# Desilo/liberate-fhe

Measured on AMD Instinct MI355X. Metric: NTTs/sec (forward negacyclic poly-NTT, logN=16, L=30 limbs, bit-exact vs reference semantics), higher is better.
Workload: dtype int64; 1 GPU; gold preset (logN=16), rows 9..38 of the prime chain (25 scale + base + 4 special primes = 30 limbs), 128 polynomials per GPU per step, forward NTT via lf_ntt_ws (C ABI: lf_ntt through a resident workspace of the operands' size); workspace_bytes=2013511680, batch_per_gpu=128, limbs=30, logN=16, parallelism=replicas x1 (independent polynomials)

## Files before the change

### include/ckks_hip.h

```cpp
#ifndef CKKS_HIP_H
#define CKKS_HIP_H

#include <stdint.h>

#ifdef __cplusplus
extern "C" {
#endif

#define LF_ERR_ARG 10001
#define LF_ERR_STATE 10002

#define LF_ABI_VERSION 15
int lf_abi_version(void);

#define LF_LIMIT_DIGIT_LIMBS 0
#define LF_LIMIT_SPECIAL_PRIMES 1
#define LF_LIMIT_ROWS 2
#define LF_LIMIT_BATCH 3
#define LF_LIMIT_LOGN 4
int lf_limits(int which);

#define LF_FP64_MAX_DIGITS 119

#define LF_BSGS_MAX_BABY_KEYS 63


#define LF_TUNE_KS_EXT_COLS_MAX 1
#define LF_TUNE_INTT_DIGITS 2
#define LF_TUNE_DIGIT_PLANES 3
#define LF_TUNE_WS_EXTRA_STAGE 4
#define LF_TUNE_MORE_PLANES 5
#define LF_TUNE_PC_MATMUL_TILE 6
int lf_tune(int which, int value);

int lf_clock_probe(uint64_t *out, int samples, uint64_t ticks, int device, void *stream);


int lf_mont_mult(const int64_t *a, const int64_t *b, int64_t *c, int rows, int64_t N,
                 const int64_t *ql, const int64_t *qh, const int64_t *kl, const int64_t *kh,
                 int device, void *stream);

int lf_mont_enter(int64_t *a, const int64_t *Rs, int rows, int64_t N,
                  const int64_t *ql, const int64_t *qh, const int64_t *kl, const int64_t *kh,
                  int device, void *stream);

int lf_mont_redc(int64_t *a, int rows, int64_t N,
                 const int64_t *ql, const int64_t *qh, const int64_t *kl, const int64_t *kh,
                 int device, void *stream);

int lf_reduce_2q(int64_t *a, int rows, int64_t N, const int64_t *_2q, int device, void *stream);
int lf_make_signed(int64_t *a, int rows, int64_t N, const int64_t *_2q, int device, void *stream);
int lf_make_unsigned(int64_t *a, int rows, int64_t N, const int64_t *_2q, int device, void *stream);
int lf_tile_unsigned(const int64_t *a, int64_t *dst, int rows, int64_t N, const int64_t *_2q,
                     int device, void *stream);
int lf_mont_add(const int64_t *a, const int64_t *b, int64_t *c, int rows, int64_t N, const int64_t *_2q,
// ... 347 lines not shown
```

### liberate_fhe_amd/csrc/ckks_common.h

```cpp
#pragma once
#include <hip/hip_runtime.h>
#include <stdint.h>

typedef long long i64;
typedef unsigned long long u64;
typedef unsigned __int128 u128;
typedef __int128 i128;

#define M62 ((1ull << 62) - 1ull)

#define KS_MAX_ALPHA 8
#define KS_MAX_K 8
#define MAX_LIST_ROWS 250
#define LF_BATCH_MAX 8
#define NTT_TILE_LOG_MAX 12
#define KS_LOGN_MAX (NTT_TILE_LOG_MAX + 5)


static __device__ __forceinline__ i64 mm62s(i64 a, i64 b, u64 q, u64 k) {
    const i128 x = (i128)a * (i128)b;
    const u64 lo = (u64)x;
    const i64 hi = (i64)(x >> 64);
    const u64 xl = lo & M62;
    const i64 xh = (i64)(((u64)hi << 2) | (lo >> 62));
// ... 80 lines not shown
#define DP_MAGIC 4503599627370496.0
static __device__ __forceinline__ double dp_from_word(i64 x) {
    return __longlong_as_double(x | 0x4330000000000000ll) - DP_MAGIC;
}
static __device__ __forceinline__ i64 dp_to_word(double d) {
    return __double_as_longlong(d + DP_MAGIC) & 0x000FFFFFFFFFFFFFll;
}

static __device__ __forceinline__ double dp_from_planes(unsigned lo, unsigned hi16) {
    return __longlong_as_double((i64)(((u64)(0x43300000u | hi16) << 32) | (u64)lo)) - DP_MAGIC;
}
typedef unsigned lf_u4_t __attribute__((ext_vector_type(4)));
typedef unsigned lf_u2_t __attribute__((ext_vector_type(2)));

static __device__ __forceinline__ double dp_from_signed(i64 x) {
    return __longlong_as_double(x + 0x4338000000000000ll) - 6755399441055744.0;
}


#define LF_FMT_RAW 0
#define LF_FMT_PLANES 1
#define LF_FMT_WS_SPLIT0 2
#define LF_FMT_WS_SPLIT1 3
void lf_fmt_note(const void *p, size_t bytes, int fmt);
void lf_fmt_epoch_bump(int fmt);
int lf_fmt_expect(const void *p, size_t bytes, int fmt);

static inline int lf_set_device(int device) {
    if (device >= 0) {
        hipError_t e = hipSetDevice(device);
        if (e != hipSuccess) return (int)e;
    }
    return 0;
}
```

### liberate_fhe_amd/csrc/ckks_hip.hip

```cpp
#include <mutex>
#include "../../include/ckks_hip.h"
#include "ckks_common.h"

namespace {


enum EwOp { EW_MULT, EW_ENTER, EW_REDC, EW_REDUCE, EW_SIGNED, EW_UNSIGNED, EW_TILE, EW_ADD, EW_SUB };

template <int OP>
__global__ void __launch_bounds__(256) ew_kernel(const i64 *a, const i64 *__restrict__ b, i64 *c,
                                                 i64 N, const i64 *__restrict__ v0, const i64 *__restrict__ ql,
                                                 const i64 *__restrict__ qh, const i64 *__restrict__ kl,
                                                 const i64 *__restrict__ kh) {
    const int row = blockIdx.y;
    const i64 j = ((i64)blockIdx.x * 256 + threadIdx.x) * 2;
    if (j >= N) return;
    const i64 off = (i64)row * N + j;
    u64 q = 0, k = 0;
    i64 q2 = 0, sc = 0;
    if (OP == EW_MULT || OP == EW_ENTER || OP == EW_REDC) {
        q = ((u64)qh[row] << 31) | (u64)ql[row];
        k = ((u64)kh[row] << 31) | (u64)kl[row];
    }
    if (OP == EW_ENTER) sc = v0[row];
// ... 79 lines not shown
        out[2 * i] = c1 - c0;
        out[2 * i + 1] = r1 - r0;
    }
}

}

namespace {
struct FmtRange {
    uintptr_t lo, hi;
    int fmt;
    unsigned long long age;
    unsigned epoch;
};
std::mutex g_fmt_mutex;
FmtRange g_fmt[256];
int g_fmt_n = 0;
unsigned long long g_fmt_clock = 0;
unsigned g_fmt_epoch[2] = {0, 0};
}

void lf_fmt_epoch_bump(int fmt) {
    std::lock_guard<std::mutex> lock(g_fmt_mutex);
    ++g_fmt_epoch[(fmt >> 1) & 1];
}

void lf_fmt_note(const void *p, size_t bytes, int fmt) {
    if (!p || !bytes) return;
    const uintptr_t lo = (uintptr_t)p, hi = lo + bytes;
    std::lock_guard<std::mutex> lock(g_fmt_mutex);
    int n = 0;
    for (int i = 0; i < g_fmt_n; ++i) {
        FmtRange r = g_fmt[i];
        if (r.hi <= lo || r.lo >= hi) {
            g_fmt[n++] = r;
            continue;
        }
        if (r.lo < lo) {
            r.hi = lo;
            g_fmt[n++] = r;
        } else if (r.hi > hi) {
            r.lo = hi;
            g_fmt[n++] = r;
        }
    }
    g_fmt_n = n;
    if (g_fmt_n == 256) {
        int o = 0;
        for (int i = 1; i < 256; ++i)
            if (g_fmt[i].age < g_fmt[o].age) o = i;
        g_fmt[o] = g_fmt[--g_fmt_n];
    }
    g_fmt[g_fmt_n++] = FmtRange{lo, hi, fmt, ++g_fmt_clock, g_fmt_epoch[(fmt >> 1) & 1]};
}

int lf_fmt_expect(const void *p, size_t bytes, int fmt) {
    if (!p || !bytes) return 0;
    const uintptr_t lo = (uintptr_t)p, hi = lo + bytes;
    std::lock_guard<std::mutex> lock(g_fmt_mutex);
    const int fam = (fmt >> 1) & 1;
    for (int i = 0; i < g_fmt_n; ++i)
        if (g_fmt[i].hi > lo && g_fmt[i].lo < hi && g_fmt[i].fmt != fmt && ((g_fmt[i].fmt >> 1) & 1) == fam &&
            g_fmt[i].epoch != g_fmt_epoch[fam])
            return LF_ERR_STATE;
    return 0;
}

extern "C" {

int lf_abi_version(void) { return LF_ABI_VERSION; }

int lf_clock_probe(uint64_t *out, int samples, uint64_t ticks, int device, void *stream) {
    if (!out || samples < 1 || samples > 4096 || ticks < 1 || ticks > 100000000ull || (uint64_t)samples * ticks > 1000000000ull)
        return LF_ERR_ARG;
    if (int e = lf_set_device(device)) return e;
    hipLaunchKernelGGL(clock_probe_kernel, dim3(1), dim3(64), 0, (hipStream_t)stream, (unsigned long long *)out, samples,
                       (unsigned long long)ticks);
    return (int)hipGetLastError();
}

int lf_limits(int which) {
    switch (which) {
        case LF_LIMIT_DIGIT_LIMBS: return KS_MAX_ALPHA;
        case LF_LIMIT_SPECIAL_PRIMES: return KS_MAX_K;
        case LF_LIMIT_ROWS: return MAX_LIST_ROWS;
// ... 91 lines not shown
```

### liberate_fhe_amd/csrc/ckks_ks.hip

```cpp
#include "../../include/ckks_hip.h"
#include "ckks_ntt_core.h"
#include "ckks_ntt_tile16.h"

#define KS_WORDS ((1 << NTT_TILE_LOG_MAX) / NTT_THREADS)

#define KS_ST(p, v)                                                  \
    do {                                                             \
        if (NT_KS_EXT) __builtin_nontemporal_store((i64)(v), p);     \
        else *(p) = (v);                                             \
    } while (0)

#define KS_ST_PL(rowb, N, idx, v)                                                                                \
    do {                                                                                                         \
        const i64 v_ = (i64)(v);                                                                                 \
        unsigned *lo_ = uniform_at(reinterpret_cast<unsigned *>(rowb) + (idx), lane);                            \
        unsigned short *hi_ = uniform_at(reinterpret_cast<unsigned short *>((rowb) + ((N) >> 1)) + (idx), lane); \
        if (NT_KS_EXT) {                                                                                         \
            __builtin_nontemporal_store((unsigned)v_, lo_);                                                      \
            __builtin_nontemporal_store((unsigned short)(v_ >> 32), hi_);                                        \
        } else {                                                                                                 \
            *lo_ = (unsigned)v_;                                                                                 \
            *hi_ = (unsigned short)(v_ >> 32);                                                                   \
        }                                                                                                        \
    } while (0)
// ... 3030 lines not shown
    }
    const dim3 grid((unsigned)((((i64)1 << logN) + 511) / 512), (unsigned)rows);
    const bool planes = key_format == LF_KEY_PLANES;
#define LF_BABYB_LAUNCH(NCT, PL, DPLB)                                                                                         \
    hipLaunchKernelGGL((ks_inner_babyb_kernel<NCT, PL, DPLB>), grid, dim3(256), 0, st, (const i64 *)ext, ba, (i64)part_stride, \
                       (i64)comp_stride, (i64)row_off, nparts, rows, logN, (const i64 *)ql, (const i64 *)qh, (const i64 *)kl,  \
                       (const i64 *)kh)
#define LF_BABYB_CASE(NCT)                                                                                                   \
    if (planes && dplanes) LF_BABYB_LAUNCH(NCT, true, true);                                                                 \
    else if (planes) LF_BABYB_LAUNCH(NCT, true, false);                                                                      \
    else if (dplanes) LF_BABYB_LAUNCH(NCT, false, true);                                                                     \
    else LF_BABYB_LAUNCH(NCT, false, false)
    if (nct == 2) {
        LF_BABYB_CASE(2);
    } else {
        LF_BABYB_CASE(4);
    }
#undef LF_BABYB_LAUNCH
#undef LF_BABYB_CASE
    return (int)hipGetLastError();
}

int lf_g_intt_digits = 1;
extern int lf_g_ws_extra_stage;

extern "C" {

int lf_tune(int which, int value) {
    int *knob = which == LF_TUNE_KS_EXT_COLS_MAX ? &g_ks_ext_cols_max : which == LF_TUNE_INTT_DIGITS ? &lf_g_intt_digits
                : which == LF_TUNE_DIGIT_PLANES ? &g_digit_planes : which == LF_TUNE_WS_EXTRA_STAGE ? &lf_g_ws_extra_stage
                : which == LF_TUNE_MORE_PLANES ? &g_more_planes : which == LF_TUNE_PC_MATMUL_TILE ? &g_pc_matmul_tile : nullptr;
    if (!knob) return -1;
    const int old = *knob;
    if (value < 0) return old;
    if (which == LF_TUNE_KS_EXT_COLS_MAX && value > 5) return old;
    if (which == LF_TUNE_MORE_PLANES && value > 3) return old;
    if (which == LF_TUNE_PC_MATMUL_TILE && value > 2) return old;
    if ((which == LF_TUNE_INTT_DIGITS || which == LF_TUNE_DIGIT_PLANES || which == LF_TUNE_WS_EXTRA_STAGE) && value > 1) return old;
    if (*knob != value && (which == LF_TUNE_DIGIT_PLANES || which == LF_TUNE_WS_EXTRA_STAGE || which == LF_TUNE_MORE_PLANES))
        lf_fmt_epoch_bump(which == LF_TUNE_WS_EXTRA_STAGE ? LF_FMT_WS_SPLIT0 : LF_FMT_RAW);
    *knob = value;
    return old;
}

int lf_key_planes(const int64_t *src_b, const int64_t *src_a, int64_t *dst_b, int64_t *dst_a, int rows, int64_t N,
                  const int64_t *ql, const int64_t *qh, int device, void *stream) {
    if (rows < 0 || rows > 65535 || N < 2 || (N & 1) || !src_b || !src_a || !dst_b || !dst_a || dst_b == dst_a || src_b == dst_b ||
        src_a == dst_a || src_a == dst_b || src_b == dst_a || !ql || !qh ||
        (((uintptr_t)src_b | (uintptr_t)src_a | (uintptr_t)dst_b | (uintptr_t)dst_a) & 15))
        return LF_ERR_ARG;
    if (rows == 0) return 0;
    if (int e = lf_set_device(device)) return e;
    hipLaunchKernelGGL(key_planes_kernel, dim3((unsigned)((N / 2 + 255) / 256), (unsigned)rows), dim3(256), 0, (hipStream_t)stream,
                       (const i64 *)src_b, (const i64 *)src_a, (i64 *)dst_b, (i64 *)dst_a, (i64)N, (const i64 *)ql, (const i64 *)qh);
    return (int)hipGetLastError();
}

int lf_ks_core_batch(const int64_t *state, int64_t state_stride, int nct, int nparts, int rows, int logN, const int64_t *desc,
                     const int64_t *E, const double *Ed, const int64_t *ksk, int64_t part_stride, int64_t comp_stride,
                     int64_t row_off, int key_format, int64_t *tmp, int64_t *s, const int64_t *psi_br, const double *psi_dp,
                     const int64_t *ipsi_br, const double *ipsi_dp, const int64_t *Ninv, const int64_t *q_host, const int64_t *ql, const int64_t *qh, const int64_t *kl, const int64_t *kh, int device,
                     void *stream) {
    if (nparts < 1 || rows < 1 || rows > MAX_LIST_ROWS || logN <= NTT_TILE_LOG_MAX || logN > KS_LOGN_MAX ||
// ... 98 lines not shown
```

### liberate_fhe_amd/csrc/ckks_ntt.hip

```cpp
#include <utility>
#include "../../include/ckks_hip.h"
#include "ckks_ntt_core.h"
#include "ckks_ntt_tile16.h"
#include <stdlib.h>

int lf_g_ws_extra_stage = 1;

namespace {

void classify(int rows, const int64_t *q_host, const void *dp_table, RowList &dp, RowList &in) {
    dp.n = in.n = 0;
    for (int r = 0; r < rows; ++r) {
        const bool small = q_host && dp_table && (uint64_t)q_host[r] < SMALL_PRIME_LIMIT;
        RowList &dst = small ? dp : in;
        dst.id[dst.n++] = (unsigned short)r;
    }
}

template <bool DP>
void launch_cols(int K, unsigned blocks, hipStream_t st, i64 *base, const PassGeom &g, const RowList &rl,
                 const int64_t *psi_br, const double *psi_dp, const i64 *rs, const int64_t *ql, const int64_t *qh,
                 const int64_t *kl, const int64_t *kh) {
#define LF_COLS_CASE(KK)                                                                                              \
    case KK:                                                                                                          \
        hipLaunchKernelGGL((ntt_fwd_cols<DP, KK>), dim3(blocks), dim3(NTT_COL_THREADS), 0, st, base, g, rl,           \
                           (const i64 *)psi_br, psi_dp, rs, (const i64 *)ql, (const i64 *)qh, (const i64 *)kl,        \
                           (const i64 *)kh);                                                                          \
        break;
    switch (K) {
// ... 254 lines not shown
    for (int pass = (S1 > 0 ? 0 : 1); pass < 2; ++pass) {
        if (only_pass && pass + 1 != only_pass) continue;
        PassGeom g = pass == 0 ? PassGeom{logN, tl, 1, S1, 0, tl - S1, rows, nb, relaxed, 0, plain}
                               : PassGeom{logN, tl, 0, tl, S1, 0, rows, nb, relaxed, 1, plain};
        const i64 *rs = (pass == 0 || S1 == 0) ? (const i64 *)Rs : nullptr;
        if (xpl) {
            const size_t bytes = ((size_t)nb * rows << logN) * 8;
            if (pass == 0) {
                g.pln = PLN_OUT;
                lf_fmt_note(base, bytes, LF_FMT_PLANES);
            } else if (int e = lf_fmt_expect(base, bytes, LF_FMT_PLANES)) {
                return e;
            }
        } else if (rsrc && relaxed && plain) {
            const size_t bytes = ((size_t)nb * rows << logN) * 8;
            if (pass == 0) lf_fmt_note(base, bytes, LF_FMT_RAW);
            else if (int e = lf_fmt_expect(base, bytes, LF_FMT_RAW)) return e;
        }
        if (through_ws) {
            const bool extra = lf_g_ws_extra_stage && S1 <= 4;
            const int Kc = S1 + (extra ? 1 : 0);
            {
                const size_t bytes = ((size_t)nb * rows << logN) * 8;
                const int fmt = extra ? LF_FMT_WS_SPLIT1 : LF_FMT_WS_SPLIT0;
                if (pass == 0) lf_fmt_note(ws, bytes, fmt);
                else if (int e = lf_fmt_expect(ws, bytes, fmt)) return e;
            }
            if (pass == 0) {
                const unsigned per_limb = (unsigned)nb * ((1u << (logN - Kc)) / NTT_COL_THREADS);
                const ClassLists cl = class_lists(in, dp, per_limb * (unsigned)in.n);
                const unsigned blocks = (unsigned)cl.in_blocks + per_limb * (unsigned)dp.n;
                switch (Kc) {
                    case 1: launch_cols_ws_k<1>(blocks, st, base, (i64 *)ws, wflags, g, cl, psi_br, psi_dp, rs, ql, qh, kl, kh); break;
                    case 2: launch_cols_ws_k<2>(blocks, st, base, (i64 *)ws, wflags, g, cl, psi_br, psi_dp, rs, ql, qh, kl, kh); break;
                    case 3: launch_cols_ws_k<3>(blocks, st, base, (i64 *)ws, wflags, g, cl, psi_br, psi_dp, rs, ql, qh, kl, kh); break;
                    case 4: launch_cols_ws_k<4>(blocks, st, base, (i64 *)ws, wflags, g, cl, psi_br, psi_dp, rs, ql, qh, kl, kh); break;
                    case 5: launch_cols_ws_k<5>(blocks, st, base, (i64 *)ws, wflags, g, cl, psi_br, psi_dp, rs, ql, qh, kl, kh); break;
                }
            } else {
                launch_pass16_ws(nb, st, (const i64 *)ws, wflags, base, g, in, dp, (const i64 *)psi_br, psi_dp, (const i64 *)ql,
                                 (const i64 *)qh, (const i64 *)kl, (const i64 *)kh, extra);
            }
            continue;
        }
        if (pass == 0 && (S1 <= 4 || (S1 == 5 && rsrc))) {
            const unsigned col_blocks = (unsigned)nb * ((1u << (logN - S1)) / NTT_COL_THREADS);
            if (rsrc) {
// ... 194 lines not shown
```

### liberate_fhe_amd/csrc/ckks_ntt_core.h

```cpp
#pragma once
#include "ckks_common.h"
#include <stdlib.h>

#define NTT_THREADS 512
#define NTT_PASS_WAVES 6
#define NTT_LDS_WORDS ((1 << NTT_TILE_LOG_MAX) + (1 << (NTT_TILE_LOG_MAX - 3)))
#define TAIL_NONE (-1)
#define SMALL_PRIME_LIMIT (1ull << 41)

#define PAD(L) ((L) + ((L) >> 3))
#define PAD_STRIDE(LOGDL) ((1 << (LOGDL)) + ((1 << (LOGDL)) >> 3))
#define NTT_FLAG_WORD NTT_LDS_WORDS

namespace {

__device__ __forceinline__ int lf_tid() {
    const int wave = __builtin_amdgcn_readfirstlane((int)threadIdx.x >> 6);
    int lane;
    asm volatile("v_mbcnt_lo_u32_b32 %0, -1, 0\n\tv_mbcnt_hi_u32_b32 %0, -1, %0" : "=v"(lane));
    return (wave << 6) | lane;
}

__device__ __forceinline__ void lds_barrier() {
    asm volatile("s_waitcnt lgkmcnt(0)" ::: "memory");
// ... 10 lines not shown
}

struct RowList {
    int n;
    unsigned short id[MAX_LIST_ROWS];
};

struct PassGeom {
    int logN;
    int tl;
    int strided;
    int S;
    int s0;
    int logC;
    int rows;
    int batch;
    int relaxed;
    int last;
    int plain;
    const unsigned char *skip_own;
    int skip_mod, skip_off;
    int pln;
    const i64 *pln_src;
};
#define PLN_IN 1
#define PLN_OUT 2

__device__ __forceinline__ int tile_gaddr(const PassGeom &g, int tile, int L) {
    if (!g.strided) return (tile << g.tl) + L;
    const int r = L >> g.logC, c = L & ((1 << g.logC) - 1);
    return (r << (g.logN - g.S)) + (tile << g.logC) + c;
}

__device__ __forceinline__ void block_coords(const PassGeom &g, const RowList &rl, int b, int &poly, int &limb, int &tile) {
    const int tiles = 1 << (g.logN - g.tl);
    const int pairs = rl.n * tiles;
    int pair;
    if ((pairs & 7) == 0) {
        const int x = b & 7, r = b >> 3;
        poly = r % g.batch;
        pair = (r / g.batch) * 8 + x;
    } else {
        pair = b / g.batch;
        poly = b % g.batch;
    }
    limb = rl.id[pair / tiles];
    tile = pair % tiles;
// ... 120 lines not shown
    const ShoupW *tw_sh;
    int relaxed;
    int inv_reduce;
};

template <bool DP>
__device__ __forceinline__ void set_aux(Ctx &c, const double *aux, int crow, int logN) {
    const double *row = aux ? aux + ((i64)crow << (logN + 1)) : nullptr;
    c.tw_dp = DP ? row : nullptr;
    c.tw_sh = DP ? nullptr : reinterpret_cast<const ShoupW *>(row);
}

template <bool SIGNED>
struct ArithInt {
    typedef i64 T;
    typedef i64 W;
    static __device__ __forceinline__ W tw(const Ctx &c, int idx) { return c.tw_mont[(unsigned)idx]; }
    template <int MAXC>
    static __device__ __forceinline__ void tw_group(const Ctx &c, int idx0, int cnt, W (&w)[MAXC]) { load_group<MAXC>(c.tw_mont, idx0, cnt, w); }
    static __device__ __forceinline__ T mul(const Ctx &c, W S, T O) {
        return SIGNED ? mm62s(S, O, c.m.q, c.m.k) : mm62u((u64)S, (u64)O, c.m.q, c.m.k);
    }
    static __device__ __forceinline__ void fwd(const Ctx &c, T &a, T &b, W S, int) {
        const T U = a, V = mul(c, S, b);
        if constexpr (SIGNED) {
            a = csub(U + V, c.m.q2);
            b = csub(U + c.m.q2 - V, c.m.q2);
        } else {
            a = (T)csub_u((u64)U + (u64)V, (u64)c.m.q2);
            b = (T)sub_lazy_u((u64)U, (u64)V, (u64)c.m.q2);
        }
    }
    static __device__ __forceinline__ void inv(const Ctx &c, T &a, T &b, W S, int) {
        const T U = a, V = b;
        if constexpr (SIGNED) {
            const T O = csub(U + c.m.q2 - V, c.m.q2);
            b = mul(c, S, O);
            a = csub(U + V, c.m.q2);
        } else {
            const T O = (T)sub_lazy_u((u64)U, (u64)V, (u64)c.m.q2);
            b = mul(c, S, O);
            a = (T)csub_u((u64)U + (u64)V, (u64)c.m.q2);
        }
    }
    template <int NN>
    static __device__ __forceinline__ void fwd_end(const Ctx &, T (&)[NN]) {}
    template <int NN>
// ... 918 lines not shown
                                                 unsigned char *__restrict__ wflags, const PassGeom &g, const RowList &rl,
                                                 const i64 *__restrict__ psi_br, const double *__restrict__ psi_dp,
                                                 const i64 *__restrict__ Rs, const i64 *__restrict__ ql,
                                                 const i64 *__restrict__ qh, const i64 *__restrict__ kl,
                                                 const i64 *__restrict__ kh) {
    constexpr int R = 1 << K;
    const int logC = g.logN - K;
    const int chunks = (1 << logC) / NTT_COL_THREADS;
    const int chunk = b % chunks, r = b / chunks;
    const int poly = __builtin_amdgcn_readfirstlane(r % g.batch), crow = __builtin_amdgcn_readfirstlane((int)rl.id[r / g.batch]);
    const bool enter = Rs != nullptr;
    Ctx c;
    c.m = load_mod(ql, qh, kl, kh, crow);
    c.tw_mont = psi_br + ((i64)crow << g.logN);
    set_aux<DP>(c, psi_dp, crow, g.logN);
    c.d = DP ? make_dp_tab(c.m, c.tw_dp) : make_dp(c.m);
    c.relaxed = 0;
    c.inv_reduce = 0;
    const i64 rs = enter ? Rs[crow] : 0;
    const i64 ri = (i64)(poly * g.rows + crow);
    const i64 col0 = (i64)chunk * NTT_COL_THREADS;
    const i64 *colu = a + (ri << g.logN) + col0;
    const unsigned lane = threadIdx.x;
    i64 w[R];
#pragma unroll
    for (int k = 0; k < R; ++k) w[k] = __builtin_nontemporal_load(uniform_at(colu + ((i64)k << logC), lane));
    int odd = 0;
#pragma unroll
    for (int k = 0; k < R; ++k) odd |= ((u64)w[k] >= (u64)c.m.q2);
    if (DP && !odd) {
        double x[R];
        const double r1 = enter ? (double)((1ull << 62) % c.m.q) : 0.0;
#pragma unroll
        for (int k = 0; k < R; ++k) {
            double v = dp_from_word(w[k]);
            if (enter) {
                v = dp_mulmod(v, r1, c.d);
                if (dp_below_fix_limit(v)) v = dp_lazy_fix(v, (u64)w[k], (u64)rs, c.d.q);
            }
            x[k] = v;
        }
        cols_fwd_stages<ArithDp, K>(x, c);
#pragma unroll
        for (int k = 0; k < R; ++k) w[k] = dp_to_word(dp_reduce(x[k], c.d.q2, c.d.q2inv));
    } else {
        if (enter) {
#pragma unroll
            for (int k = 0; k < R; ++k) {
                w[k] = mm62s(w[k], rs, c.m.q, c.m.k);
                odd |= ((u64)w[k] >= (u64)c.m.q2);
            }
        }
        if (odd || DP) cols_fwd_stages<ArithInt<true>, K>(w, c);
        else cols_fwd_stages<ArithInt<false>, K>(w, c);
    }
    i64 *orow = ws + (ri << g.logN);
    const bool wide = __builtin_amdgcn_ballot_w64(odd != 0) != 0;
    if ((lane & 63u) == 0) {
        const unsigned c0 = (unsigned)col0 + lane;
        wflags[(ri << 6) + (((c0 >> 6) & 3u) << 4) + (c0 >> 8)] = wide ? 1 : 0;
    }
    if constexpr (!DP) {
        const unsigned ls = lane_here(lane, orow);
#pragma unroll
        for (int k = 0; k < R; ++k) __builtin_nontemporal_store(w[k], uniform_at(orow + col0 + ((i64)k << logC), ls));
    } else {
        unsigned *lo = reinterpret_cast<unsigned *>(orow) + col0;
        unsigned short *mid = reinterpret_cast<unsigned short *>(orow + ((i64)1 << (g.logN - 1))) + col0;
#pragma unroll
        for (int k = 0; k < R; ++k) __builtin_nontemporal_store((unsigned)w[k], uniform_at(lo + ((i64)k << logC), lane));
#pragma unroll
        for (int k = 0; k < R; ++k)
            __builtin_nontemporal_store((unsigned short)((u64)w[k] >> 32), uniform_at(mid + ((i64)k << logC), lane));
        if (wide) {
            unsigned short *top = reinterpret_cast<unsigned short *>(orow + 3 * ((i64)1 << (g.logN - 2))) + col0;
#pragma unroll
            for (int k = 0; k < R; ++k) top[((i64)k << logC) + lane] = (unsigned short)((u64)w[k] >> 48);
// ... 480 lines not shown
```

### liberate_fhe_amd/csrc/ckks_ntt_tile16.h

```cpp
#pragma once
#include "ckks_ntt_core.h"

#define NTT16_THREADS 256
#define PAD16(L) ((L) + ((L) >> 4))
#define NTT16_LDS_WORDS (4096 + 256)
#define NTT16_FLAG NTT16_LDS_WORDS

namespace {

template <class A>
struct Tw16Early {
    typename A::W w1[1], w2[2], w4[4];
    __device__ __forceinline__ void load(const Ctx &c, int i) {
        A::tw_group(c, i, 1, w1);
        A::tw_group(c, i << 1, 2, w2);
        A::tw_group(c, i << 2, 4, w4);
    }
    __device__ __forceinline__ void get(int cnt, typename A::W (&wv)[8]) const {
#pragma unroll
        for (int j = 0; j < 4; ++j)
            if (j < cnt) wv[j] = cnt == 1 ? w1[0] : (cnt == 2 ? w2[j & 1] : w4[j]);
    }
};

template <class A>
struct Tw16Last {
    typename A::W w8[8];
    __device__ __forceinline__ void load(const Ctx &c, int i) { A::tw_group(c, i << 3, 8, w8); }
};

template <class A, int U0 = 0>
__device__ __forceinline__ void fwd_regs16(typename A::T (&x)[16], int i0, const Ctx &c, const Tw16Early<A> *early = nullptr,
                                           const Tw16Last<A> *last = nullptr) {
#pragma unroll
    for (int u = U0; u < 4; ++u) {
        const int du = 1 << (3 - u);
        typename A::W wv[8];
        if (early && u < 3) early->get(1 << u, wv);
        else if (last && u == 3) {
#pragma unroll
            for (int j = 0; j < 8; ++j) wv[j] = last->w8[j];
        } else A::tw_group(c, i0 << u, 1 << u, wv);
#pragma unroll
        for (int j = 0; j < (1 << u); ++j) {
            const int e0 = j << (4 - u);
#pragma unroll
            for (int t = 0; t < du; ++t) A::fwd(c, x[e0 + t], x[e0 + t + du], wv[j], (i0 << u) + j);
        }
    }
    A::fwd_end(c, x);
}

template <int U0 = 0>
__device__ __forceinline__ void fwd_regs16_exact(double (&x)[16], int i0, const Ctx &c, const Tw16Early<ArithDp> *early = nullptr,
                                                 const Tw16Last<ArithDp> *last = nullptr) {
#pragma unroll
    for (int u = U0; u < 4; ++u) {
        const int du = 1 << (3 - u);
        double wv[8];
        if (early && u < 3) early->get(1 << u, wv);
        else if (last && u == 3) {
#pragma unroll
            for (int j = 0; j < 8; ++j) wv[j] = last->w8[j];
        } else ArithDp::tw_group(c, i0 << u, 1 << u, wv);
        double V[8];
#pragma unroll
        for (int j = 0; j < (1 << u); ++j) {
            const int e0 = j << (4 - u);
#pragma unroll
            for (int t = 0; t < du; ++t) V[j * du + t] = dp_mulmod(x[e0 + t + du], wv[j], c.d);
        }
        int hmin = min(min(__double2hiint(V[0]), __double2hiint(V[1])), __double2hiint(V[2]));
        hmin = min(min(hmin, __double2hiint(V[3])), __double2hiint(V[4]));
        hmin = min(min(hmin, __double2hiint(V[5])), __double2hiint(V[6]));
        hmin = min(hmin, __double2hiint(V[7]));
        if (__builtin_expect(__builtin_amdgcn_ballot_w64(hmin < 0x41500000) != 0, 0)) {
#pragma unroll
            for (int j = 0; j < (1 << u); ++j) {
                const int e0 = j << (4 - u);
#pragma unroll
                for (int t = 0; t < du; ++t) {
// ... 63 lines not shown
                for (int t = 0; t < du; ++t) {
                    const int k = h * du + t;
                    if (dp_below_fix_limit(V[k]))
                        V[k] = dp_lazy_fix(V[k], (u64)c.tw_mont[(il << (3 - u)) + h], (u64)dp_reduce(O[k], c.d.q2, c.d.q2inv), c.d.q);
                }
            }
        }
#pragma unroll
        for (int h = 0; h < (1 << (3 - u)); ++h) {
            const int e0 = h << (u + 1);
#pragma unroll
            for (int t = 0; t < du; ++t) {
                const int k = h * du + t;
                x[e0 + t] = x[e0 + t] + x[e0 + t + du];
                x[e0 + t + du] = V[k];
            }
        }
    }
#pragma unroll
    for (int e = 0; e < 16; ++e) x[e] = dp_reduce(x[e], c.d.q2, c.d.q2inv);
}

__device__ __forceinline__ void tile16_slow_compute(i64 *sm, int base, int s0, int logN, bool inverse, const Ctx &c, int j0 = 0,
                                                    int j1 = 12) {
    for (int j = j0; j < j1; ++j) {
        const int st = s0 + j;
        const int logd = inverse ? j : 11 - j;
        for (int i = threadIdx.x; i < 2048; i += NTT16_THREADS) {
            const int pa = ((i >> logd) << (logd + 1)) | (i & ((1 << logd) - 1)), pb = pa + (1 << logd);
            i64 a = sm[PAD16(pa)], b = sm[PAD16(pb)];
            if (!inverse) {
                const int idx = (1 << st) + ((base + pa) >> (logN - st));
                ArithInt<true>::fwd(c, a, b, c.tw_mont[idx], idx);
            } else {
                const int idx = (1 << (logN - st - 1)) + ((base + pa) >> (st + 1));
                ArithInt<true>::inv(c, a, b, c.tw_mont[idx], idx);
            }
            sm[PAD16(pa)] = a;
            sm[PAD16(pb)] = b;
        }
        __syncthreads();
    }
}
__device__ __forceinline__ void tile16_slow_lds(i64 *sm, i64 *dst, int base, int s0, int logN, bool inverse, const Ctx &c, int j0 = 0,
                                                int j1 = 12) {
    tile16_slow_compute(sm, base, s0, logN, inverse, c, j0, j1);
    for (int L = threadIdx.x; L < 4096; L += NTT16_THREADS) dst[L] = sm[PAD16(L)];
}
__device__ __forceinline__ void tile16_slow(i64 *sm, const i64 *src, i64 *dst, int base, int s0, int logN, bool inverse, const Ctx &c) {
    for (int L = threadIdx.x; L < 4096; L += NTT16_THREADS) sm[PAD16(L)] = src[L];
    __syncthreads();
    tile16_slow_lds(sm, dst, base, s0, logN, inverse, c);
}

__device__ __forceinline__ void wave_flag_set16(i64 *sm, int pred, int w) {
    const bool any = __builtin_amdgcn_ballot_w64(pred != 0) != 0;
    if ((w & 63) == 0) reinterpret_cast<unsigned char *>(sm + NTT16_FLAG)[w >> 6] = any ? 1 : 0;
}
__device__ __forceinline__ bool tile_flagged16(const i64 *sm) { return reinterpret_cast<const unsigned *>(sm + NTT16_FLAG)[0] != 0; }

template <bool RLX> struct DpArith { typedef ArithDp type; };
template <> struct DpArith<true> { typedef ArithDpR type; };

template <class A, bool EXACT_DP, int U0 = 0>
__device__ __forceinline__ void fwd_step16(typename A::T (&x)[16], int i0, const Ctx &c, const Tw16Early<A> *early,
                                           const Tw16Last<A> *last = nullptr) {
    if constexpr (EXACT_DP) fwd_regs16_exact<U0>(x, i0, c, early, last);
    else fwd_regs16<A, U0>(x, i0, c, early, last);
}
template <class A, bool EXACT_DP>
__device__ __forceinline__ void inv_step16(typename A::T (&x)[16], int il, const Ctx &c, const Tw16Early<A> *early) {
    if constexpr (EXACT_DP) inv_regs16_exact(x, il, c, early);
    else inv_regs16<A>(x, il, c, early);
}

template <class A, bool DP, bool RLX, int U0 = 0>
__device__ __forceinline__ bool fwd_tile16_steps(typename A::T *smt, const i64 *sm, typename A::T (&x)[16], int w, int base,
                                                 int E, int s, const Ctx &c, bool check, const Tw16Last<A> *lastC = nullptr) {
    constexpr bool EX = DP && !RLX;
    const int iA = (1 << s) + (base >> (E - s));
    const int pB = ((w >> 4) << 8) | (w & 15);
    const int iB = (1 << (s + 4)) + ((base + pB) >> (E - s - 4));
    const int iC = (1 << (s + 8)) + ((base + 16 * w) >> (E - s - 8));
    Tw16Early<A> twB, twC;
    fwd_step16<A, EX, U0>(x, iA, c, nullptr);
    {
        typename A::T *sp = smt + PAD16(w);
#pragma unroll
        for (int e = 0; e < 16; ++e) sp[e * 272] = x[e];
    }
    twB.load(c, iB);
    lds_barrier();
    if (check && tile_flagged16(sm)) return false;
    {
        typename A::T *sp = smt + PAD16(pB);
#pragma unroll
        for (int e = 0; e < 16; ++e) x[e] = sp[e * 17];
        fwd_step16<A, EX>(x, iB, c, &twB);
#pragma unroll
        for (int e = 0; e < 16; ++e) sp[e * 17] = x[e];
    }
    twC.load(c, iC);
    lds_barrier();
    {
        const typename A::T *sp = smt + 17 * w;
#pragma unroll
        for (int e = 0; e < 16; ++e) x[e] = sp[e];
    }
// ... 127 lines not shown
            const unsigned l = __builtin_nontemporal_load(uniform_at(lo + (e << 8), (unsigned)w));
            const unsigned m = __builtin_nontemporal_load(uniform_at(mid + (e << 8), (unsigned)w));
            raw[e] = (i64)(((u64)m << 32) | (u64)l);
        }
        if ((fl | fh) != 0) {
            const unsigned short *top = reinterpret_cast<const unsigned short *>(srow + 3 * ((i64)1 << (E - 2))) + base;
#pragma unroll
            for (int e = 0; e < 16; ++e)
                if ((((e < 8 ? fl : fh) >> (8 * (e & 7))) & 0xffull) != 0) raw[e] |= (i64)((u64)top[(e << 8) + w] << 48);
        }
    } else {
#pragma unroll
        for (int e = 0; e < 16; ++e) raw[e] = __builtin_nontemporal_load(uniform_at(srow + base + (e << 8), (unsigned)w));
    }
    return (fl | fh) != 0;
}

template <bool DP, bool SKIP0>
__device__ __forceinline__ void fwd_tile16_ws(i64 *sm, const i64 *__restrict__ srow, const unsigned char *__restrict__ wf,
                                              i64 *__restrict__ row, int tile, const PassGeom &g, const Ctx &c,
                                              const Tw16Last<typename FwdArith<DP, false>::type> *lastC = nullptr) {
    const int w = lf_tid();
    const int base = tile << 12, E = g.logN, s = g.s0;
    i64 raw[16];
    const bool flagged = ws_load_tile<DP, SKIP0>(srow, wf, base, E, w, raw);
    {
        int odd = 0;
        if (flagged) {
#pragma unroll
            for (int e = 0; e < 16; ++e) odd |= ((u64)raw[e] >= (u64)c.m.q2);
        }
        wave_flag_set16(sm, odd, w);
    }
    i64 o[16];
    bool ok;
    if constexpr (DP) {
        double x[16];
#pragma unroll
        for (int e = 0; e < 16; ++e) x[e] = dp_from_word(raw[e]);
        ok = fwd_tile16_steps<ArithDp, true, false, SKIP0 ? 1 : 0>(reinterpret_cast<double *>(sm), sm, x, w, base, E, s, c, true, lastC);
#pragma unroll
        for (int e = 0; e < 16; ++e) o[e] = dp_to_word(dp_reduce(x[e], c.d.q2, c.d.q2inv));
    } else {
        ok = fwd_tile16_steps<ArithInt<false>, false, false, SKIP0 ? 1 : 0>(sm, sm, raw, w, base, E, s, c, true, lastC);
#pragma unroll
        for (int e = 0; e < 16; ++e) o[e] = raw[e];
    }
    if (!ok) {
        __syncthreads();
        ws_load_tile<DP, SKIP0>(srow, wf, base, E, w, raw);
#pragma unroll
        for (int e = 0; e < 16; ++e) sm[PAD16(w + (e << 8))] = raw[e];
        __syncthreads();
        tile16_slow_lds(sm, row + base, base, s, E, false, c, SKIP0 ? 1 : 0);
        return;
    }
    {
        i64 *sp = sm + 17 * w;
#pragma unroll
        for (int e = 0; e < 16; ++e) sp[e] = o[e];
    }
    wave_lds_sync();
    const int L0 = ((w >> 6) << 10) + ((w & 63) << 1);
    const i64 *so = sm + PAD16(L0);
#pragma unroll
    for (int i = 0; i < 8; ++i) {
        longlong2 v;
        v.x = so[i * 136];
        v.y = so[i * 136 + 1];
        if constexpr (NT_EXACT) nt_store2(row + base + L0 + (i << 7), v);
        else *reinterpret_cast<longlong2 *>(row + base + L0 + (i << 7)) = v;
    }
}

template <class A, bool DP, bool RLX>
__device__ __forceinline__ bool inv_tile16_steps(typename A::T *smt, const i64 *sm, typename A::T (&x)[16], int w, int base,
                                                 int logN, int s, const Ctx &c, bool check) {
// ... 448 lines not shown
    const u64 fl = fp[0], fh = SKIP0 ? fp[0] : fp[1];
    if constexpr (DP) {
        const unsigned *lo = reinterpret_cast<const unsigned *>(srow) + base;
        const unsigned short *mid = reinterpret_cast<const unsigned short *>(srow + ((i64)1 << (E - 1))) + base;
#pragma unroll
        for (int e = 0; e < 16; ++e) {
            pf.lo[e] = __builtin_nontemporal_load(uniform_at(lo + (e << 8), (unsigned)w));
            pf.mid[e] = __builtin_nontemporal_load(uniform_at(mid + (e << 8), (unsigned)w));
        }
    } else {
#pragma unroll
        for (int e = 0; e < 16; ++e) pf.raw[e] = __builtin_nontemporal_load(uniform_at(srow + base + (e << 8), (unsigned)w));
    }
    return (fl | fh) != 0;
}

template <bool DP, bool SKIP0>
__device__ __forceinline__ void fwd_tile16_ws_pf(i64 *sm, TilePf<DP> &pf, bool &pf_flagged, const i64 *__restrict__ srow,
                                                  const unsigned char *__restrict__ wf, i64 *__restrict__ row, int tile,
                                                  const PassGeom &g, const Ctx &c, const Tw16Last<typename FwdArith<DP, false>::type> *lastC,
                                                  const i64 *__restrict__ nsrow, const unsigned char *__restrict__ nwf, int ntile) {
    const int w = lf_tid();
    const int base = tile << 12, E = g.logN, s = g.s0;
    i64 raw[16];
    const bool flagged = pf_flagged;
    if (flagged) {
        ws_load_tile<DP, SKIP0>(srow, wf, base, E, w, raw);
    } else if constexpr (DP) {
#pragma unroll
        for (int e = 0; e < 16; ++e) raw[e] = (i64)(((u64)pf.mid[e] << 32) | (u64)pf.lo[e]);
    } else {
#pragma unroll
        for (int e = 0; e < 16; ++e) raw[e] = pf.raw[e];
    }
    {
        int odd = 0;
        if (flagged) {
#pragma unroll
            for (int e = 0; e < 16; ++e) odd |= ((u64)raw[e] >= (u64)c.m.q2);
        }
        wave_flag_set16(sm, odd, w);
    }
    i64 o[16];
    bool ok;
    if constexpr (DP) {
        double x[16];
#pragma unroll
        for (int e = 0; e < 16; ++e) x[e] = dp_from_word(raw[e]);
        ok = fwd_tile16_steps<ArithDp, true, false, SKIP0 ? 1 : 0>(reinterpret_cast<double *>(sm), sm, x, w, base, E, s, c, true, lastC);
#pragma unroll
        for (int e = 0; e < 16; ++e) o[e] = dp_to_word(dp_reduce(x[e], c.d.q2, c.d.q2inv));
    } else {
        ok = fwd_tile16_steps<ArithInt<false>, false, false, SKIP0 ? 1 : 0>(sm, sm, raw, w, base, E, s, c, true, lastC);
#pragma unroll
        for (int e = 0; e < 16; ++e) o[e] = raw[e];
    }
    if (!ok) {
        __syncthreads();
        ws_load_tile<DP, SKIP0>(srow, wf, base, E, w, raw);
#pragma unroll
        for (int e = 0; e < 16; ++e) sm[PAD16(w + (e << 8))] = raw[e];
        __syncthreads();
        tile16_slow_lds(sm, row + base, base, s, E, false, c, SKIP0 ? 1 : 0);
        if (ntile >= 0) pf_flagged = ws_prefetch_tile<DP, SKIP0>(nsrow, nwf, ntile << 12, E, w, pf);
        else pf = TilePf<DP>{};
        return;
    }

    {
        i64 *sp = sm + 17 * w;
#pragma unroll
        for (int e = 0; e < 16; ++e) sp[e] = o[e];
    }
    __builtin_amdgcn_sched_barrier(0);
    if (ntile >= 0) pf_flagged = ws_prefetch_tile<DP, SKIP0>(nsrow, nwf, ntile << 12, E, w, pf);
    else pf = TilePf<DP>{};
    __builtin_amdgcn_sched_barrier(0);
    wave_lds_sync();
    const int L0 = ((w >> 6) << 10) + ((w & 63) << 1);
    const i64 *so = sm + PAD16(L0);
#pragma unroll
    for (int i = 0; i < 8; ++i) {
        longlong2 v;
        v.x = so[i * 136];
        v.y = so[i * 136 + 1];
        if constexpr (NT_EXACT) nt_store2(row + base + L0 + (i << 7), v);
// ... 219 lines not shown
```

Before: 82460 poly-NTT/s.

## Premultiply extra-stage twiddles in column pass to skip tile's first twiddle multiply

When the workspace split includes an extra stage, the column pass now multiplies its outputs by the next stage's twiddle factors (both the DP and integer paths), so the tile16 pass can run its first butterfly stage as plain add/sub without a modular multiply. A new tune knob selects this per arithmetic path, and the workspace format tag encodes the premultiplied variant so stale workspaces are rejected. This moves the twiddle multiply from the register-heavy tile kernel into the column kernel, which adds twiddle loads and a fix-up path there.

Result: no change. 83180 poly-NTT/s (median of 3 runs) (+0.9%).

```diff
diff --git a/include/ckks_hip.h b/include/ckks_hip.h
--- a/include/ckks_hip.h
+++ b/include/ckks_hip.h
@@ -31,6 +31,7 @@
 #define LF_TUNE_WS_EXTRA_STAGE 4
 #define LF_TUNE_MORE_PLANES 5
 #define LF_TUNE_PC_MATMUL_TILE 6
+#define LF_TUNE_WS_PREMUL 7
 int lf_tune(int which, int value);
 
 int lf_clock_probe(uint64_t *out, int samples, uint64_t ticks, int device, void *stream);
diff --git a/liberate_fhe_amd/csrc/ckks_common.h b/liberate_fhe_amd/csrc/ckks_common.h
--- a/liberate_fhe_amd/csrc/ckks_common.h
+++ b/liberate_fhe_amd/csrc/ckks_common.h
@@ -126,6 +126,7 @@
 #define LF_FMT_PLANES 1
 #define LF_FMT_WS_SPLIT0 2
 #define LF_FMT_WS_SPLIT1 3
+#define LF_FMT_FAMILY(fmt) ((fmt) >= LF_FMT_WS_SPLIT0 ? 1 : 0)
 void lf_fmt_note(const void *p, size_t bytes, int fmt);
 void lf_fmt_epoch_bump(int fmt);
 int lf_fmt_expect(const void *p, size_t bytes, int fmt);
diff --git a/liberate_fhe_amd/csrc/ckks_hip.hip b/liberate_fhe_amd/csrc/ckks_hip.hip
--- a/liberate_fhe_amd/csrc/ckks_hip.hip
+++ b/liberate_fhe_amd/csrc/ckks_hip.hip
@@ -125,7 +125,7 @@
 
 void lf_fmt_epoch_bump(int fmt) {
     std::lock_guard<std::mutex> lock(g_fmt_mutex);
-    ++g_fmt_epoch[(fmt >> 1) & 1];
+    ++g_fmt_epoch[LF_FMT_FAMILY(fmt)];
 }
 
 void lf_fmt_note(const void *p, size_t bytes, int fmt) {
@@ -154,16 +154,16 @@
             if (g_fmt[i].age < g_fmt[o].age) o = i;
         g_fmt[o] = g_fmt[--g_fmt_n];
     }
-    g_fmt[g_fmt_n++] = FmtRange{lo, hi, fmt, ++g_fmt_clock, g_fmt_epoch[(fmt >> 1) & 1]};
+    g_fmt[g_fmt_n++] = FmtRange{lo, hi, fmt, ++g_fmt_clock, g_fmt_epoch[LF_FMT_FAMILY(fmt)]};
 }
 
 int lf_fmt_expect(const void *p, size_t bytes, int fmt) {
     if (!p || !bytes) return 0;
     const uintptr_t lo = (uintptr_t)p, hi = lo + bytes;
     std::lock_guard<std::mutex> lock(g_fmt_mutex);
-    const int fam = (fmt >> 1) & 1;
+    const int fam = LF_FMT_FAMILY(fmt);
     for (int i = 0; i < g_fmt_n; ++i)
-        if (g_fmt[i].hi > lo && g_fmt[i].lo < hi && g_fmt[i].fmt != fmt && ((g_fmt[i].fmt >> 1) & 1) == fam &&
+        if (g_fmt[i].hi > lo && g_fmt[i].lo < hi && g_fmt[i].fmt != fmt && LF_FMT_FAMILY(g_fmt[i].fmt) == fam &&
             g_fmt[i].epoch != g_fmt_epoch[fam])
             return LF_ERR_STATE;
     return 0;
diff --git a/liberate_fhe_amd/csrc/ckks_ks.hip b/liberate_fhe_amd/csrc/ckks_ks.hip
--- a/liberate_fhe_amd/csrc/ckks_ks.hip
+++ b/liberate_fhe_amd/csrc/ckks_ks.hip
@@ -3076,23 +3076,25 @@
 }
 
 int lf_g_intt_digits = 1;
-extern int lf_g_ws_extra_stage;
+extern int lf_g_ws_extra_stage, lf_g_ws_premul;
 
 extern "C" {
 
 int lf_tune(int which, int value) {
     int *knob = which == LF_TUNE_KS_EXT_COLS_MAX ? &g_ks_ext_cols_max : which == LF_TUNE_INTT_DIGITS ? &lf_g_intt_digits
                 : which == LF_TUNE_DIGIT_PLANES ? &g_digit_planes : which == LF_TUNE_WS_EXTRA_STAGE ? &lf_g_ws_extra_stage
-                : which == LF_TUNE_MORE_PLANES ? &g_more_planes : which == LF_TUNE_PC_MATMUL_TILE ? &g_pc_matmul_tile : nullptr;
+                : which == LF_TUNE_MORE_PLANES ? &g_more_planes : which == LF_TUNE_PC_MATMUL_TILE ? &g_pc_matmul_tile
+                : which == LF_TUNE_WS_PREMUL ? &lf_g_ws_premul : nullptr;
     if (!knob) return -1;
     const int old = *knob;
     if (value < 0) return old;
     if (which == LF_TUNE_KS_EXT_COLS_MAX && value > 5) return old;
-    if (which == LF_TUNE_MORE_PLANES && value > 3) return old;
+    if ((which == LF_TUNE_MORE_PLANES || which == LF_TUNE_WS_PREMUL) && value > 3) return old;
     if (which == LF_TUNE_PC_MATMUL_TILE && value > 2) return old;
     if ((which == LF_TUNE_INTT_DIGITS || which == LF_TUNE_DIGIT_PLANES || which == LF_TUNE_WS_EXTRA_STAGE) && value > 1) return old;
-    if (*knob != value && (which == LF_TUNE_DIGIT_PLANES || which == LF_TUNE_WS_EXTRA_STAGE || which == LF_TUNE_MORE_PLANES))
-        lf_fmt_epoch_bump(which == LF_TUNE_WS_EXTRA_STAGE ? LF_FMT_WS_SPLIT0 : LF_FMT_RAW);
+    const bool ws_knob = which == LF_TUNE_WS_EXTRA_STAGE || which == LF_TUNE_WS_PREMUL;
+    if (*knob != value && (which == LF_TUNE_DIGIT_PLANES || ws_knob || which == LF_TUNE_MORE_PLANES))
+        lf_fmt_epoch_bump(ws_knob ? LF_FMT_WS_SPLIT0 : LF_FMT_RAW);
     *knob = value;
     return old;
 }
diff --git a/liberate_fhe_amd/csrc/ckks_ntt.hip b/liberate_fhe_amd/csrc/ckks_ntt.hip
--- a/liberate_fhe_amd/csrc/ckks_ntt.hip
+++ b/liberate_fhe_amd/csrc/ckks_ntt.hip
@@ -5,6 +5,7 @@
 #include <stdlib.h>
 
 int lf_g_ws_extra_stage = 1;
+int lf_g_ws_premul = 1;
 
 namespace {
 
@@ -305,7 +306,8 @@
             const int Kc = S1 + (extra ? 1 : 0);
             {
                 const size_t bytes = ((size_t)nb * rows << logN) * 8;
-                const int fmt = extra ? LF_FMT_WS_SPLIT1 : LF_FMT_WS_SPLIT0;
+                g.ws_premul = extra ? (lf_g_ws_premul & 3) : 0;
+                const int fmt = extra ? LF_FMT_WS_SPLIT1 + g.ws_premul : LF_FMT_WS_SPLIT0;
                 if (pass == 0) lf_fmt_note(ws, bytes, fmt);
                 else if (int e = lf_fmt_expect(ws, bytes, fmt)) return e;
             }
diff --git a/liberate_fhe_amd/csrc/ckks_ntt_core.h b/liberate_fhe_amd/csrc/ckks_ntt_core.h
--- a/liberate_fhe_amd/csrc/ckks_ntt_core.h
+++ b/liberate_fhe_amd/csrc/ckks_ntt_core.h
@@ -56,7 +56,9 @@
     int skip_mod, skip_off;
     int pln;
     const i64 *pln_src;
+    int ws_premul;
 };
+__device__ __forceinline__ bool ws_premul_on(const PassGeom &g, bool dp) { return ((g.ws_premul >> (dp ? 0 : 1)) & 1) != 0; }
 #define PLN_IN 1
 #define PLN_OUT 2
 
@@ -223,7 +225,11 @@
         return SIGNED ? mm62s(S, O, c.m.q, c.m.k) : mm62u((u64)S, (u64)O, c.m.q, c.m.k);
     }
     static __device__ __forceinline__ void fwd(const Ctx &c, T &a, T &b, W S, int) {
-        const T U = a, V = mul(c, S, b);
+        b = mul(c, S, b);
+        fwd_sums(c, a, b);
+    }
+    static __device__ __forceinline__ void fwd_sums(const Ctx &c, T &a, T &b) {
+        const T U = a, V = b;
         if constexpr (SIGNED) {
             a = csub(U + V, c.m.q2);
             b = csub(U + c.m.q2 - V, c.m.q2);
@@ -1188,6 +1194,7 @@
     const i64 col0 = (i64)chunk * NTT_COL_THREADS;
     const i64 *colu = a + (ri << g.logN) + col0;
     const unsigned lane = threadIdx.x;
+    const bool premul = ws_premul_on(g, DP) && (((unsigned)col0 >> (logC - 1)) & 1u) != 0;
     i64 w[R];
 #pragma unroll
     for (int k = 0; k < R; ++k) w[k] = __builtin_nontemporal_load(uniform_at(colu + ((i64)k << logC), lane));
@@ -1207,8 +1214,38 @@
             x[k] = v;
         }
         cols_fwd_stages<ArithDp, K>(x, c);
-#pragma unroll
-        for (int k = 0; k < R; ++k) w[k] = dp_to_word(dp_reduce(x[k], c.d.q2, c.d.q2inv));
+        if (premul) {
+            constexpr int G = R < 8 ? R : 8;
+            double tw[G];
+            load_group<G>(c.tw_dp, R, G, tw);
+#pragma unroll
+            for (int k0 = 0; k0 < R; k0 += G) {
+                double tn[G], V[G];
+                if (k0 + G < R) load_group<G>(c.tw_dp, R + k0 + G, G, tn);
+                int hmin = 0x7fffffff;
+#pragma unroll
+                for (int j = 0; j < G; ++j) {
+                    V[j] = dp_mulmod(x[k0 + j], tw[j], c.d);
+                    hmin = min(hmin, __double2hiint(V[j]));
+                }
+                if (__builtin_expect(__builtin_amdgcn_ballot_w64(hmin < 0x41500000) != 0, 0)) {
+#pragma unroll
+                    for (int j = 0; j < G; ++j)
+                        if (dp_below_fix_limit(V[j]))
+                            V[j] = dp_lazy_fix(V[j], (u64)c.tw_mont[R + k0 + j], (u64)dp_reduce(x[k0 + j], c.d.q2, c.d.q2inv), c.d.q);
+                }
+#pragma unroll
+                for (int j = 0; j < G; ++j) {
+                    x[k0 + j] = V[j];
+                    if (k0 + G < R) tw[j] = tn[j];
+                }
+            }
+        } else {
+#pragma unroll
+            for (int k = 0; k < R; ++k) x[k] = dp_reduce(x[k], c.d.q2, c.d.q2inv);
+        }
+#pragma unroll
+        for (int k = 0; k < R; ++k) w[k] = dp_to_word(x[k]);
     } else {
         if (enter) {
 #pragma unroll
@@ -1217,8 +1254,19 @@
                 odd |= ((u64)w[k] >= (u64)c.m.q2);
             }
         }
-        if (odd || DP) cols_fwd_stages<ArithInt<true>, K>(w, c);
-        else cols_fwd_stages<ArithInt<false>, K>(w, c);
+        if (odd || DP) {
+            cols_fwd_stages<ArithInt<true>, K>(w, c);
+            if (premul) {
+#pragma unroll
+                for (int k = 0; k < R; ++k) w[k] = ArithInt<true>::mul(c, c.tw_mont[R + k], w[k]);
+            }
+        } else {
+            cols_fwd_stages<ArithInt<false>, K>(w, c);
+            if (premul) {
+#pragma unroll
+                for (int k = 0; k < R; ++k) w[k] = ArithInt<false>::mul(c, c.tw_mont[R + k], w[k]);
+            }
+        }
     }
     i64 *orow = ws + (ri << g.logN);
     const bool wide = __builtin_amdgcn_ballot_w64(odd != 0) != 0;
diff --git a/liberate_fhe_amd/csrc/ckks_ntt_tile16.h b/liberate_fhe_amd/csrc/ckks_ntt_tile16.h
--- a/liberate_fhe_amd/csrc/ckks_ntt_tile16.h
+++ b/liberate_fhe_amd/csrc/ckks_ntt_tile16.h
@@ -29,12 +29,22 @@
     __device__ __forceinline__ void load(const Ctx &c, int i) { A::tw_group(c, i << 3, 8, w8); }
 };
 
-template <class A, int U0 = 0>
+template <class A, int U0 = 0, bool PM = false>
 __device__ __forceinline__ void fwd_regs16(typename A::T (&x)[16], int i0, const Ctx &c, const Tw16Early<A> *early = nullptr,
                                            const Tw16Last<A> *last = nullptr) {
 #pragma unroll
     for (int u = U0; u < 4; ++u) {
         const int du = 1 << (3 - u);
+        if constexpr (PM) {
+            if (u == U0) {
+#pragma unroll
+                for (int j = 0; j < (1 << u); ++j) {
+#pragma unroll
+                    for (int t = 0; t < du; ++t) A::fwd_sums(c, x[(j << (4 - u)) + t], x[(j << (4 - u)) + t + du]);
+                }
+                continue;
+            }
+        }
         typename A::W wv[8];
         if (early && u < 3) early->get(1 << u, wv);
         else if (last && u == 3) {
@@ -51,12 +61,27 @@
     A::fwd_end(c, x);
 }
 
-template <int U0 = 0>
+template <int U0 = 0, bool PM = false>
 __device__ __forceinline__ void fwd_regs16_exact(double (&x)[16], int i0, const Ctx &c, const Tw16Early<ArithDp> *early = nullptr,
                                                  const Tw16Last<ArithDp> *last = nullptr) {
 #pragma unroll
     for (int u = U0; u < 4; ++u) {
         const int du = 1 << (3 - u);
+        if constexpr (PM) {
+            if (u == U0) {
+#pragma unroll
+                for (int j = 0; j < (1 << u); ++j) {
+                    const int e0 = j << (4 - u);
+#pragma unroll
+                    for (int t = 0; t < du; ++t) {
+                        const double U = x[e0 + t], Vv = x[e0 + t + du];
+                        x[e0 + t] = U + Vv;
+                        x[e0 + t + du] = U - Vv;
+                    }
+                }
+                continue;
+            }
+        }
         double wv[8];
         if (early && u < 3) early->get(1 << u, wv);
         else if (last && u == 3) {
@@ -166,7 +191,7 @@
 }
 
 __device__ __forceinline__ void tile16_slow_compute(i64 *sm, int base, int s0, int logN, bool inverse, const Ctx &c, int j0 = 0,
-                                                    int j1 = 12) {
+                                                    int j1 = 12, int jpm = -1) {
     for (int j = j0; j < j1; ++j) {
         const int st = s0 + j;
         const int logd = inverse ? j : 11 - j;
@@ -175,7 +200,8 @@
             i64 a = sm[PAD16(pa)], b = sm[PAD16(pb)];
             if (!inverse) {
                 const int idx = (1 << st) + ((base + pa) >> (logN - st));
-                ArithInt<true>::fwd(c, a, b, c.tw_mont[idx], idx);
+                if (j == jpm) ArithInt<true>::fwd_sums(c, a, b);
+                else ArithInt<true>::fwd(c, a, b, c.tw_mont[idx], idx);
             } else {
                 const int idx = (1 << (logN - st - 1)) + ((base + pa) >> (st + 1));
                 ArithInt<true>::inv(c, a, b, c.tw_mont[idx], idx);
@@ -187,8 +213,8 @@
     }
 }
 __device__ __forceinline__ void tile16_slow_lds(i64 *sm, i64 *dst, int base, int s0, int logN, bool inverse, const Ctx &c, int j0 = 0,
-                                                int j1 = 12) {
-    tile16_slow_compute(sm, base, s0, logN, inverse, c, j0, j1);
+                                                int j1 = 12, int jpm = -1) {
+    tile16_slow_compute(sm, base, s0, logN, inverse, c, j0, j1, jpm);
     for (int L = threadIdx.x; L < 4096; L += NTT16_THREADS) dst[L] = sm[PAD16(L)];
 }
 __device__ __forceinline__ void tile16_slow(i64 *sm, const i64 *src, i64 *dst, int base, int s0, int logN, bool inverse, const Ctx &c) {
@@ -206,11 +232,11 @@
 template <bool RLX> struct DpArith { typedef ArithDp type; };
 template <> struct DpArith<true> { typedef ArithDpR type; };
 
-template <class A, bool EXACT_DP, int U0 = 0>
+template <class A, bool EXACT_DP, int U0 = 0, bool PM = false>
 __device__ __forceinline__ void fwd_step16(typename A::T (&x)[16], int i0, const Ctx &c, const Tw16Early<A> *early,
                                            const Tw16Last<A> *last = nullptr) {
-    if constexpr (EXACT_DP) fwd_regs16_exact<U0>(x, i0, c, early, last);
-    else fwd_regs16<A, U0>(x, i0, c, early, last);
+    if constexpr (EXACT_DP) fwd_regs16_exact<U0, PM>(x, i0, c, early, last);
+    else fwd_regs16<A, U0, PM>(x, i0, c, early, last);
 }
 template <class A, bool EXACT_DP>
 __device__ __forceinline__ void inv_step16(typename A::T (&x)[16], int il, const Ctx &c, const Tw16Early<A> *early) {
@@ -220,14 +246,20 @@
 
 template <class A, bool DP, bool RLX, int U0 = 0>
 __device__ __forceinline__ bool fwd_tile16_steps(typename A::T *smt, const i64 *sm, typename A::T (&x)[16], int w, int base,
-                                                 int E, int s, const Ctx &c, bool check, const Tw16Last<A> *lastC = nullptr) {
+                                                 int E, int s, const Ctx &c, bool check, const Tw16Last<A> *lastC = nullptr,
+                                                 bool premul = false) {
     constexpr bool EX = DP && !RLX;
     const int iA = (1 << s) + (base >> (E - s));
     const int pB = ((w >> 4) << 8) | (w & 15);
     const int iB = (1 << (s + 4)) + ((base + pB) >> (E - s - 4));
     const int iC = (1 << (s + 8)) + ((base + 16 * w) >> (E - s - 8));
     Tw16Early<A> twB, twC;
-    fwd_step16<A, EX, U0>(x, iA, c, nullptr);
+    if constexpr (U0 == 1 && !RLX) {
+        if (premul) fwd_step16<A, EX, U0, true>(x, iA, c, nullptr);
+        else fwd_step16<A, EX, U0>(x, iA, c, nullptr);
+    } else {
+        fwd_step16<A, EX, U0>(x, iA, c, nullptr);
+    }
     {
         typename A::T *sp = smt + PAD16(w);
 #pragma unroll
@@ -401,6 +433,7 @@
                                               const Tw16Last<typename FwdArith<DP, false>::type> *lastC = nullptr) {
     const int w = lf_tid();
     const int base = tile << 12, E = g.logN, s = g.s0;
+    const bool premul = SKIP0 && ws_premul_on(g, DP);
     i64 raw[16];
     const bool flagged = ws_load_tile<DP, SKIP0>(srow, wf, base, E, w, raw);
     {
@@ -417,11 +450,11 @@
         double x[16];
 #pragma unroll
         for (int e = 0; e < 16; ++e) x[e] = dp_from_word(raw[e]);
-        ok = fwd_tile16_steps<ArithDp, true, false, SKIP0 ? 1 : 0>(reinterpret_cast<double *>(sm), sm, x, w, base, E, s, c, true, lastC);
+        ok = fwd_tile16_steps<ArithDp, true, false, SKIP0 ? 1 : 0>(reinterpret_cast<double *>(sm), sm, x, w, base, E, s, c, true, lastC, premul);
 #pragma unroll
         for (int e = 0; e < 16; ++e) o[e] = dp_to_word(dp_reduce(x[e], c.d.q2, c.d.q2inv));
     } else {
-        ok = fwd_tile16_steps<ArithInt<false>, false, false, SKIP0 ? 1 : 0>(sm, sm, raw, w, base, E, s, c, true, lastC);
+        ok = fwd_tile16_steps<ArithInt<false>, false, false, SKIP0 ? 1 : 0>(sm, sm, raw, w, base, E, s, c, true, lastC, premul);
 #pragma unroll
         for (int e = 0; e < 16; ++e) o[e] = raw[e];
     }
@@ -431,7 +464,7 @@
 #pragma unroll
         for (int e = 0; e < 16; ++e) sm[PAD16(w + (e << 8))] = raw[e];
         __syncthreads();
-        tile16_slow_lds(sm, row + base, base, s, E, false, c, SKIP0 ? 1 : 0);
+        tile16_slow_lds(sm, row + base, base, s, E, false, c, SKIP0 ? 1 : 0, 12, premul ? 1 : -1);
         return;
     }
     {
@@ -926,6 +959,7 @@
                                                   const i64 *__restrict__ nsrow, const unsigned char *__restrict__ nwf, int ntile) {
     const int w = lf_tid();
     const int base = tile << 12, E = g.logN, s = g.s0;
+    const bool premul = SKIP0 && ws_premul_on(g, DP);
     i64 raw[16];
     const bool flagged = pf_flagged;
     if (flagged) {
@@ -951,11 +985,11 @@
         double x[16];
 #pragma unroll
         for (int e = 0; e < 16; ++e) x[e] = dp_from_word(raw[e]);
-        ok = fwd_tile16_steps<ArithDp, true, false, SKIP0 ? 1 : 0>(reinterpret_cast<double *>(sm), sm, x, w, base, E, s, c, true, lastC);
+        ok = fwd_tile16_steps<ArithDp, true, false, SKIP0 ? 1 : 0>(reinterpret_cast<double *>(sm), sm, x, w, base, E, s, c, true, lastC, premul);
 #pragma unroll
         for (int e = 0; e < 16; ++e) o[e] = dp_to_word(dp_reduce(x[e], c.d.q2, c.d.q2inv));
     } else {
-        ok = fwd_tile16_steps<ArithInt<false>, false, false, SKIP0 ? 1 : 0>(sm, sm, raw, w, base, E, s, c, true, lastC);
+        ok = fwd_tile16_steps<ArithInt<false>, false, false, SKIP0 ? 1 : 0>(sm, sm, raw, w, base, E, s, c, true, lastC, premul);
 #pragma unroll
         for (int e = 0; e < 16; ++e) o[e] = raw[e];
     }
@@ -965,7 +999,7 @@
 #pragma unroll
         for (int e = 0; e < 16; ++e) sm[PAD16(w + (e << 8))] = raw[e];
         __syncthreads();
-        tile16_slow_lds(sm, row + base, base, s, E, false, c, SKIP0 ? 1 : 0);
+        tile16_slow_lds(sm, row + base, base, s, E, false, c, SKIP0 ? 1 : 0, 12, premul ? 1 : -1);
         if (ntile >= 0) pf_flagged = ws_prefetch_tile<DP, SKIP0>(nsrow, nwf, ntile << 12, E, w, pf);
         else pf = TilePf<DP>{};
         return;
```
